# hmorimitsu/ptlflow

Measured on NVIDIA B200. Metric: frame-pairs/sec RAFT 1024x436 12-iter, higher is better.
Workload: dtype f16 storage, f32 accumulate/coordinates

## Files before the change

### include/ptlflow_b200.h

```cpp
#ifndef PTLFLOW_B200_H_
#define PTLFLOW_B200_H_

#include <stddef.h>
#include <stdint.h>

#ifdef __cplusplus
extern "C" {
#endif

#if defined(__GNUC__)
#define PFB_API __attribute__((visibility("default")))
#else
#define PFB_API
#endif

typedef void* pfb_stream;

typedef enum { PFB_F32 = 0, PFB_F16 = 1, PFB_BF16 = 2 } pfb_dtype;

typedef enum {
  PFB_OK = 0,
  PFB_ERR_ARG = -1,
  PFB_ERR_CUDA = -2,
  PFB_ERR_UNSUPPORTED = -3
// ... 156 lines not shown
} pfb_raft_weights;

typedef struct {
  void* const* pyramid;
  const void* fmap1;
  void* net;
  const void* inp;
  float* coords;
  float* flow_up;
  float* flow_small;
  void* workspace;
  size_t workspace_bytes;
  const void* attention;
  float agg_gamma;
} pfb_raft_buffers;

PFB_API size_t pfb_raft_workspace_bytes(const pfb_raft_cfg* cfg);
PFB_API int pfb_raft_refine(const pfb_raft_cfg* cfg, const pfb_raft_weights* w, const pfb_raft_buffers* buf,
                    pfb_stream stream);
PFB_API int pfb_raft_update_iter(const pfb_raft_cfg* cfg, const pfb_raft_weights* w, const pfb_raft_buffers* buf,
                         const void* corr, void* mask_out, pfb_stream stream);

PFB_API int pfb_preprocess_frames(const void* images, void* out, int B, int H, int W, int Hp, int Wp, int pad_top,
                                  int pad_left, int out_channels, pfb_dtype dtype, pfb_stream stream);
PFB_API size_t pfb_instance_norm_workspace_bytes(int B, int C);
PFB_API int pfb_instance_norm_act(const void* x, void* y, const void* residual, void* workspace, int B, int H, int W, int C,
                                  float eps, int relu, pfb_dtype dtype, pfb_stream stream);
PFB_API int pfb_instance_norm_apply(const void* x, void* y, const void* residual, void* workspace, int B, int H, int W, int C,
                                    float eps, int relu, pfb_dtype dtype, pfb_stream stream);
PFB_API int pfb_flow_conv7x7(const float* flow, const void* wpack, const float* bias, void* out, int out_stride, int out_offset,
                             int B, int H, int W, pfb_dtype dtype, pfb_stream stream);
PFB_API int pfb_first_conv7x7s2(const void* x, const void* wpack, const float* bias, void* out, double* stats, int N, int H, int W,
                                int relu, pfb_dtype dtype, pfb_stream stream);
PFB_API int pfb_bias_act(const void* x, const float* bias, const void* residual, void* y, void* workspace, int B, int H, int W,
                         int C, int relu, pfb_dtype dtype, pfb_stream stream);

#define PFB_KERNEL_CLASSES 12
PFB_API unsigned long long pfb_launch_count(int kernel_class);
PFB_API int pfb_profile_enable(int on);
PFB_API int pfb_profile_collect(double* ms, unsigned long long* n, int len);

#ifdef __cplusplus
}
#endif
#endif
```

### ptlflow_b200/_lib.py

```python
from __future__ import annotations

import ctypes as C
import threading
import os
from typing import Optional

import torch

_PKG = os.path.dirname(os.path.abspath(__file__))
LIB_PATH = os.path.join(_PKG, "lib", "libptlflow_b200.so")

PFB_MAX_LEVELS = 8
PFB_MAX_SRC = 4

F32, F16, BF16 = 0, 1, 2
_DTYPES = {torch.float32: F32, torch.float16: F16, torch.bfloat16: BF16}

EPI_LINEAR, EPI_RELU, EPI_GRU_ZR, EPI_GRU_Q, EPI_FLOW, EPI_RELU_APPEND_FLOW, EPI_AXPY, EPI_LINEAR_F32 = range(8)

(L_CONVC1, L_CONVC2, L_CONVF1, L_CONVF2, L_CONV, L_GRU_ZR1, L_GRU_Q1, L_GRU_ZR2, L_GRU_Q2,
 L_FLOW1, L_FLOW2, L_MASK1, L_MASK2, L_AGG_V, L_FLOW2T,
 L_CTX_ZR1, L_CTX_Q1, L_CTX_ZR2, L_CTX_Q2, L_GRUX_ZR1, L_GRUX_Q1, L_GRUX_ZR2, L_GRUX_Q2, L_CONVC2F2, L_COUNT) = range(25)


# ... 59 lines not shown
    "pfb_corr_volume_build": (_I, [_P, _P, _PP, _I, _I, _I, _I, _I, _I, _I, _S]),
    "pfb_corr_volume_build_ex": (_I, [_P, _P, _PP, _I, _I, _I, _I, _I, _I, _I, C.c_float, _I, _I, _S]),
    "pfb_corr_level_bytes": (C.c_size_t, [_I, _I, _I, _I, _I]),
    "pfb_corr_lookup": (_I, [_PP, _P, _P, _I, _I, _I, _I, _I, _I, _I, _I, _I, _S]),
    "pfb_corr_lookup_ex": (_I, [_PP, C.POINTER(C.c_int), C.POINTER(C.c_int), _P, _P, _I, _I, _I, _I, _I, _I, _I, _I, _I, _S]),
    "pfb_corr_level_bytes_tiled": (C.c_size_t, [_I, _I, _I, _I, _I, _I]),
    "pfb_corr_volume_build_tiled": (_I, [_P, _P, _PP, _I, _I, _I, _I, _I, _I, _I, C.c_float, _I, _S]),
    "pfb_corr_lookup_tiled": (_I, [_PP, _P, _P, _I, _I, _I, _I, _I, _I, _I, _I, _I, _S]),
    "pfb_corr_lookup_onthefly": (_I, [_P, _PP, _P, _P, _I, _I, _I, _I, _I, _I, _I, _I, _I, _I, _S]),
    "pfb_corr_lookup_onthefly_tc_workspace_bytes": (C.c_size_t, [_I, _I, _I]),
    "pfb_corr_lookup_onthefly_tc": (_I, [_P, _PP, _P, _P, _P, _I, _I, _I, _I, _I, _I, _I, _I, _S]),
    "pfb_alt_corr_forward": (_I, [_P, _P, _P, _P, _I, _I, _I, _I, _I, _I, _I, _I, _I, _S]),
    "pfb_avg_pool2x2_nhwc": (_I, [_P, _P, _I, _I, _I, _I, _I, _S]),
    "pfb_conv2d": (_I, [C.POINTER(ConvParams), _S]),
    "pfb_pack_conv_weight": (_I, [_P, _P, _I, _I, _I, _I, _I, _I, _I, _I, _S]),
    "pfb_pack_bias": (_I, [_P, _P, _I, _I, _I, _S]),
    "pfb_pack_conv_weight_kmajor": (_I, [_P, _P, _I, _I, _I, _I, _I, _I, C.POINTER(C.c_int), _I, _I, _I, _I, _S]),
    "pfb_convex_upsample": (_I, [_P, _P, _P, _P, _I, _I, _I, _I, _I, _I, _I, _I, _S]),
    "pfb_upflow8": (_I, [_P, _P, _P, _I, _I, _I, _I, _I, _I, _I, _S]),
    "pfb_softmax_rows": (_I, [_P, C.c_size_t, _I, _I, _S]),
    "pfb_transpose_pm": (_I, [_P, _P, _I, _I, _I, _I, _I, _S]),
    "pfb_flow_tap_gather": (_I, [_P, _I, _P, _P, _P, _I, _I, _I, _S]),
    "pfb_context_split": (_I, [_P, _P, _P, _I, _I, _I, _I, _I, _I, _S]),
    "pfb_init_coords": (_I, [_P, _P, _I, _I, _I, _S]),
    "pfb_forward_interpolate": (_I, [_P, _P, _I, _I, _I, _S]),
    "pfb_raft_workspace_bytes": (C.c_size_t, [C.POINTER(RaftCfg)]),
    "pfb_raft_refine": (_I, [C.POINTER(RaftCfg), C.POINTER(RaftWeights), C.POINTER(RaftBuffers), _S]),
    "pfb_preprocess_frames": (_I, [_P, _P, _I, _I, _I, _I, _I, _I, _I, _I, _I, _S]),
    "pfb_instance_norm_workspace_bytes": (C.c_size_t, [_I, _I]),
    "pfb_instance_norm_act": (_I, [_P, _P, _P, _P, _I, _I, _I, _I, C.c_float, _I, _I, _S]),
    "pfb_instance_norm_apply": (_I, [_P, _P, _P, _P, _I, _I, _I, _I, C.c_float, _I, _I, _S]),
    "pfb_flow_conv7x7": (_I, [_P, _P, _P, _P, _I, _I, _I, _I, _I, _I, _S]),
    "pfb_first_conv7x7s2": (_I, [_P, _P, _P, _P, _P, _I, _I, _I, _I, _I, _S]),
    "pfb_bias_act": (_I, [_P, _P, _P, _P, _P, _I, _I, _I, _I, _I, _I, _S]),
    "pfb_launch_count": (C.c_ulonglong, [_I]),
    "pfb_profile_enable": (_I, [_I]),
    "pfb_profile_collect": (_I, [C.POINTER(C.c_double), C.POINTER(C.c_ulonglong), _I]),
    "pfb_raft_update_iter": (_I, [C.POINTER(RaftCfg), C.POINTER(RaftWeights), C.POINTER(RaftBuffers), _P, _P, _S]),
}


class LibraryMissing(RuntimeError):
    pass


def load() -> C.CDLL:
    global _lib
    if _lib is not None:
        return _lib
    if not os.path.exists(LIB_PATH):
        raise LibraryMissing(
            f"{LIB_PATH} not found: the ptlflow_b200 hot path is hand-written CUDA and has no fallback. "
            "Build it with `python -m ptlflow_b200.csrc.build` (needs nvcc, no GPU required to compile)."
        )
    lib = C.CDLL(LIB_PATH)
    for name, (res, args) in SIGNATURES.items():
        fn = getattr(lib, name)
        fn.restype = res
        fn.argtypes = args
    _lib = lib
    return lib


def check(rc: int, what: str = "") -> None:
    if rc != 0:
        msg = load().pfb_last_error().decode(errors="replace")
# ... 64 lines not shown
```

### ptlflow_b200/csrc/build.py

```python
from __future__ import annotations

import hashlib
import os
import subprocess
import sys
from concurrent.futures import ThreadPoolExecutor

HERE = os.path.dirname(os.path.abspath(__file__))
PKG = os.path.dirname(HERE)
ROOT = os.path.dirname(PKG)
LIB_DIR = os.path.join(PKG, "lib")
OBJ_DIR = os.path.join(HERE, "build")
LIB_PATH = os.path.join(LIB_DIR, "libptlflow_b200.so")

SOURCES = ["misc.cu", "prof.cu", "corr.cu", "conv_simt.cu", "refine.cu", "conv_umma.cu", "corr_umma.cu", "corr_tiled.cu", "corr_onthefly_umma.cu", "conv_special.cu", "tmap.cu", "encoder.cu", "first_conv.cu"]
NVCC_FLAGS = [
    "-gencode", "arch=compute_100a,code=sm_100a",
    "-O3", "-lineinfo", "-std=c++17",
    "-Xcompiler", "-fPIC", "-Xcompiler", "-fvisibility=hidden",
    "--expt-relaxed-constexpr",
]


def _nvcc() -> str:
    for cand in (os.environ.get("NVCC"), "/usr/local/cuda/bin/nvcc", "nvcc"):
        if cand and (os.path.isabs(cand) and os.path.exists(cand) or not os.path.isabs(cand)):
            return cand
    return "nvcc"


def _digest() -> str:
    h = hashlib.sha256()
    for name in sorted(os.listdir(HERE)) + [os.path.join(ROOT, "include", "ptlflow_b200.h")]:
        path = name if os.path.isabs(name) else os.path.join(HERE, name)
        if path.endswith((".cu", ".cuh", ".h", "build.py")):
            with open(path, "rb") as f:
                h.update(name.encode() + b"\0" + f.read())
    return h.hexdigest()


def build(force: bool = False, verbose: bool = False) -> str:
    os.makedirs(LIB_DIR, exist_ok=True)
    os.makedirs(OBJ_DIR, exist_ok=True)
    stamp = os.path.join(LIB_DIR, "build.stamp")
    digest = _digest()
    if not force and os.path.exists(LIB_PATH) and os.path.exists(stamp) and open(stamp).read().strip() == digest:
        return LIB_PATH
    nvcc = _nvcc()
# ... 28 lines not shown
```

### ptlflow_b200/csrc/encoder.cu

```cuda
#include <algorithm>

#include <stdlib.h>

#include "common.cuh"

namespace pfb {

template <typename T>
__global__ void preprocess_frames_kernel(const T* __restrict__ img, T* __restrict__ out, int B, int H, int W, int Hp,
                                         int Wp, int pad_top, int pad_left, int OC) {
  const size_t total = (size_t)2 * B * Hp * Wp;
  for (size_t idx = blockIdx.x * (size_t)blockDim.x + threadIdx.x; idx < total; idx += (size_t)gridDim.x * blockDim.x) {
    int x = (int)(idx % Wp);
    size_t t = idx / Wp;
    int y = (int)(t % Hp);
    int n = (int)(t / Hp);
    const int f = n / B, b = n - f * B;
    int sy = y - pad_top, sx = x - pad_left;
    sy = sy < 0 ? 0 : (sy >= H ? H - 1 : sy);
    sx = sx < 0 ? 0 : (sx >= W ? W - 1 : sx);
    const T* src = img + (((size_t)b * 2 + f) * 3) * H * W + (size_t)sy * W + sx;
    T* o = out + idx * OC;
#pragma unroll
    for (int c = 0; c < 3; ++c) {
// ... 91 lines not shown
    }
  }
  if (pl < lanes && (!pow2 || (threadIdx.x & 31) < c8n)) {
#pragma unroll
    for (int k = 0; k < 8; ++k) {
      atomicAdd(&acc[8 * co + k], s[k]);
      atomicAdd(&acc[C + 8 * co + k], q[k]);
    }
  }
  __syncthreads();
  for (int i = threadIdx.x; i < 2 * C; i += blockDim.x) {
    const int c = i % C, which = i / C;
    atomicAdd(stats + ((size_t)b * C + c) * 2 + which, (double)acc[i]);
  }
}

template <typename T>
__device__ __forceinline__ void store8(T* p, const float (&f)[8]) {
  uint4 u;
  T* h = reinterpret_cast<T*>(&u);
#pragma unroll
  for (int i = 0; i < 8; ++i) h[i] = from_f32<T>(f[i]);
  *reinterpret_cast<uint4*>(p) = u;
}
template <>
__device__ __forceinline__ void store8<float>(float* p, const float (&f)[8]) {
  reinterpret_cast<float4*>(p)[0] = make_float4(f[0], f[1], f[2], f[3]);
  reinterpret_cast<float4*>(p)[1] = make_float4(f[4], f[5], f[6], f[7]);
}

template <typename T>
__global__ void __launch_bounds__(256) affine_act_kernel(const T* __restrict__ x, const double* __restrict__ stats,
                                                         const float* __restrict__ bias, const T* __restrict__ residual,
                                                         T* __restrict__ y, int HW, int C, float eps, int relu, int pix_per_block) {
  const int b = blockIdx.y;
  const int c8n = C / 8;
  const int lanes = blockDim.x / c8n;
  const int co = threadIdx.x % c8n, pl = threadIdx.x / c8n;
  __shared__ float2 ss_sm[512];
  for (int c = threadIdx.x; c < C; c += blockDim.x) {
    float2 v = make_float2(1.f, bias ? __ldg(bias + c) : 0.f);
    if (stats) {
      const double2 sq = *reinterpret_cast<const double2*>(stats + ((size_t)b * C + c) * 2);
      const double mean = sq.x / HW;
      double var = sq.y / HW - mean * mean;
      var = var < 0 ? 0 : var;
      const float rstd = rsqrtf((float)var + eps);
      v = make_float2(rstd, (float)(-mean) * rstd);
    }
    ss_sm[c] = v;
  }
  __syncthreads();
  if (pl >= lanes) return;
  float sc[8], sh[8];
#pragma unroll
  for (int k = 0; k < 8; ++k) {
    sc[k] = ss_sm[8 * co + k].x;
    sh[k] = ss_sm[8 * co + k].y;
  }
  const int p0 = blockIdx.x * pix_per_block;
  const int p1 = min(p0 + pix_per_block, HW);
  const size_t base = (size_t)b * HW * C + 8 * co;
#pragma unroll 4
  for (int p = p0 + pl; p < p1; p += lanes) {
    const size_t off = base + (size_t)p * C;
    float v[8], r[8];
    load8<T>(x + off, v);
    if (residual) load8<T>(residual + off, r);
#pragma unroll
    for (int k = 0; k < 8; ++k) {
      float o = fmaf(v[k], sc[k], sh[k]);
      if (relu) o = fmaxf(o, 0.f);
      if (residual) o = fmaxf(r[k] + o, 0.f);
      v[k] = o;
    }
    store8<T>(y + off, v);
  }
}

template <typename T>
__global__ void __launch_bounds__(256) inorm_fused_kernel(const T* __restrict__ x, const T* __restrict__ residual, T* __restrict__ y,
                                                          double* __restrict__ stats, unsigned* __restrict__ counters, int B, int HW, int C,
                                                          float eps, int relu, int G, int ipw) {
  extern __shared__ float acc[];
  const int iw = blockIdx.x / G, g = blockIdx.x - iw * G;
  const int c8n = C / 8;
  const int lanes = blockDim.x / c8n;
  const int co = threadIdx.x % c8n, pl = threadIdx.x / c8n;
  const int slice = (HW + G - 1) / G;
  const int p0 = g * slice, p1 = min(p0 + slice, HW);
  const bool pow2 = (c8n & (c8n - 1)) == 0 && c8n <= 32 && (blockDim.x % c8n) == 0;
  for (int b = iw; b < B; b += ipw) {
    for (int i = threadIdx.x; i < 2 * C; i += blockDim.x) acc[i] = 0.f;
    __syncthreads();
    const size_t base = (size_t)b * HW * C + 8 * co;
    float s[8], q[8];
#pragma unroll
    for (int k = 0; k < 8; ++k) s[k] = q[k] = 0.f;
    if (pl < lanes) {
#pragma unroll 4
      for (int p = p0 + pl; p < p1; p += lanes) {
        float v[8];
        load8<T>(x + base + (size_t)p * C, v);
#pragma unroll
        for (int k = 0; k < 8; ++k) {
          s[k] += v[k];
// ... 77 lines not shown

extern "C" PFB_API int pfb_preprocess_frames(const void* images, void* out, int B, int H, int W, int Hp, int Wp, int pad_top,
                                             int pad_left, int out_channels, pfb_dtype dtype, pfb_stream stream) {
  PFB_CHECK_ARG(images && out, "preprocess_frames: null pointer");
  PFB_CHECK_ARG(out_channels >= 3 && out_channels <= 16, "preprocess_frames: out_channels=%d (3..16)", out_channels);
  PFB_CHECK_ARG(dtype_ok(dtype) && B > 0 && H > 0 && W > 0 && Hp >= H && Wp >= W && pad_top >= 0 && pad_left >= 0 &&
                    pad_top + H <= Hp && pad_left + W <= Wp,
                "preprocess_frames: bad geometry %dx%d -> %dx%d (+%d,+%d)", H, W, Hp, Wp, pad_top, pad_left);
  cudaStream_t s = as_stream(stream);
  size_t total = (size_t)2 * B * Hp * Wp;
  unsigned blocks = (unsigned)std::min<size_t>(ceil_div_sz(total, 256), (size_t)sm_count() * 16);
  ProfScope prof(KC_MISC, s);
  if (dtype != PFB_F32 && out_channels == 4 && pad_left == 0 && Wp == W && W % 8 == 0 &&
      ((reinterpret_cast<uintptr_t>(images) | reinterpret_cast<uintptr_t>(out)) & 15) == 0 && ((size_t)H * W) % 8 == 0) {
    blocks = (unsigned)std::min<size_t>(ceil_div_sz(total / 8, 256), (size_t)sm_count() * 16);
    if (dtype == PFB_F16) preprocess_frames_vec8_kernel<__half><<<blocks, 256, 0, s>>>((const __half*)images, (__half*)out, B, H, W, Hp, pad_top);
    else preprocess_frames_vec8_kernel<__nv_bfloat16><<<blocks, 256, 0, s>>>((const __nv_bfloat16*)images, (__nv_bfloat16*)out, B, H, W, Hp, pad_top);
    PFB_LAUNCH_CHECK();
    return PFB_OK;
  }
  PFB_DISPATCH_DTYPE(dtype, T, {
    preprocess_frames_kernel<T><<<blocks, 256, 0, s>>>((const T*)images, (T*)out, B, H, W, Hp, Wp, pad_top, pad_left, out_channels);
  });
  PFB_LAUNCH_CHECK();
  return PFB_OK;
}

extern "C" PFB_API size_t pfb_instance_norm_workspace_bytes(int B, int C) {
  return (size_t)B * C * (2 * sizeof(double) + sizeof(float2));
}

template <typename T>
static int launch_affine(const void* x, const double* stats, const float* bias, const void* residual, void* y, int B, int HW, int C,
                         float eps, int relu, cudaStream_t s) {
  const int ppb = HW >= 8192 ? 512 : (HW >= 1024 ? 128 : 32);
  dim3 grid(ceil_div(HW, ppb), B);
  affine_act_kernel<T><<<grid, 256, 0, s>>>((const T*)x, stats, bias, (const T*)residual, (T*)y, HW, C, eps, relu, ppb);
  PFB_LAUNCH_CHECK();
  return PFB_OK;
}

extern "C" PFB_API int pfb_instance_norm_act(const void* x, void* y, const void* residual, void* workspace, int B, int H, int W,
                                             int C, float eps, int relu, pfb_dtype dtype, pfb_stream stream) {
  PFB_CHECK_ARG(x && y && workspace, "instance_norm_act: null pointer");
  PFB_CHECK_ARG(dtype_ok(dtype) && B > 0 && H > 0 && W > 0 && C > 0 && C % 8 == 0 && C <= 512,
                "instance_norm_act: bad shape (C=%d must be a multiple of 8, <= 512)", C);
  cudaStream_t s = as_stream(stream);
  const int HW = H * W;
  double* stats = reinterpret_cast<double*>(workspace);
  PFB_CUDA(cudaMemsetAsync(stats, 0, (size_t)B * C * 2 * sizeof(double) + (size_t)B * sizeof(unsigned), s));
  PFB_CHECK_ARG(B <= 65535, "instance_norm_act: batch too large");
  {
    static const int env_fused = getenv("PFB_INORM_FUSED") ? atoi(getenv("PFB_INORM_FUSED")) : 0;
    const size_t image_bytes = (size_t)HW * C * dtype_size(dtype);
    if (env_fused && dtype != PFB_F32 && C <= 256 && (256 % (C / 8) == 0 || C / 8 <= 32) && HW >= 1024) {
      const size_t per_image = image_bytes * (residual ? 3 : 2);
      int ipw = (int)std::max<size_t>(1, std::min<size_t>((size_t)B, (size_t)(60u << 20) / std::max<size_t>(per_image, 1)));
      const int sms = sm_count();
      if (ipw > sms / 2) ipw = sms / 2;
      const int G = std::max(1, sms / ipw);
      unsigned* counters = reinterpret_cast<unsigned*>(stats + (size_t)B * C * 2);
      ProfScope prof(KC_ENC_AFFINE, s);
      PFB_DISPATCH_DTYPE(dtype, T, {
        inorm_fused_kernel<T><<<ipw * G, 256, 2 * C * sizeof(float), s>>>((const T*)x, (const T*)residual, (T*)y, stats, counters, B, HW, C, eps,
                                                                        relu, G, ipw);
      });
      PFB_LAUNCH_CHECK();
      return PFB_OK;
    }
  }
  const int threads = 256;
  static const int env_ppb = getenv("PFB_STATS_PPB") ? atoi(getenv("PFB_STATS_PPB")) : 0;
  const int ppb = env_ppb > 0 && HW >= 8192 ? env_ppb : (HW >= 65536 ? 1536 : (HW >= 8192 ? 768 : (HW >= 1024 ? 256 : 64)));
  dim3 grid(ceil_div(HW, ppb), B);
  {
    ProfScope prof(KC_ENC_STATS, s);
    PFB_DISPATCH_DTYPE(dtype, T, { inorm_stats_kernel<T><<<grid, threads, 2 * C * sizeof(float), s>>>((const T*)x, stats, HW, C, ppb); });
  }
  PFB_LAUNCH_CHECK();
  ProfScope prof(KC_ENC_AFFINE, s);
  PFB_DISPATCH_DTYPE(dtype, T, { return launch_affine<T>(x, stats, nullptr, residual, y, B, HW, C, eps, relu, s); });
  return PFB_OK;
}

extern "C" PFB_API int pfb_instance_norm_apply(const void* x, void* y, const void* residual, void* workspace, int B, int H, int W,
                                               int C, float eps, int relu, pfb_dtype dtype, pfb_stream stream) {
  PFB_CHECK_ARG(x && y && workspace, "instance_norm_apply: null pointer");
  PFB_CHECK_ARG(dtype_ok(dtype) && B > 0 && H > 0 && W > 0 && C > 0 && C % 8 == 0 && C <= 512 && B <= 65535,
                "instance_norm_apply: bad shape (C=%d must be a multiple of 8, <= 512)", C);
  cudaStream_t s = as_stream(stream);
  const int HW = H * W;
  double* stats = reinterpret_cast<double*>(workspace);
  ProfScope prof(KC_ENC_AFFINE, s);
  PFB_DISPATCH_DTYPE(dtype, T, { return launch_affine<T>(x, stats, nullptr, residual, y, B, HW, C, eps, relu, s); });
  return PFB_OK;
}

extern "C" PFB_API int pfb_bias_act(const void* x, const float* bias, const void* residual, void* y, void* workspace, int B, int H,
                                    int W, int C, int relu, pfb_dtype dtype, pfb_stream stream) {
  PFB_CHECK_ARG(x && y && workspace, "bias_act: null pointer");
  PFB_CHECK_ARG(dtype_ok(dtype) && B > 0 && H > 0 && W > 0 && C > 0 && C % 8 == 0 && C <= 512, "bias_act: bad shape (C=%d must be a multiple of 8, <= 512)", C);
  PFB_CHECK_ARG(B <= 65535, "bias_act: batch too large");
  cudaStream_t s = as_stream(stream);
  (void)workspace;
  ProfScope prof(KC_ENC_AFFINE, s);
  PFB_DISPATCH_DTYPE(dtype, T, { return launch_affine<T>(x, nullptr, bias, residual, y, B, H * W, C, 0.f, relu, s); });
  return PFB_OK;
}
```

### ptlflow_b200/models/raft/extractor.py

```python
from __future__ import annotations

import os
import threading

import torch
import torch.nn as nn
import torch.nn.functional as F

from ... import _lib, ops


def _norm(kind: str, channels: int, groups: int = 8) -> nn.Module:
    if kind == "batch":
        return nn.BatchNorm2d(channels)
    if kind == "instance":
        return nn.InstanceNorm2d(channels)
    if kind == "group":
        return nn.GroupNorm(num_groups=groups, num_channels=channels)
    if kind == "none":
        return nn.Identity()
    raise ValueError(f"unknown norm_fn {kind!r}")


class ResidualBlock(nn.Module):
# ... 30 lines not shown
        g = planes // 8
        self.norm1, self.norm2, self.norm3 = _norm(norm_fn, q, g), _norm(norm_fn, q, g), _norm(norm_fn, planes, g)
        self.downsample = None
        if stride != 1:
            self.norm4 = _norm(norm_fn, planes, g)
            self.downsample = nn.Sequential(nn.Conv2d(in_planes, planes, 1, stride=stride), self.norm4)

    def forward(self, x):
        y = self.relu(self.norm1(self.conv1(x)))
        y = self.relu(self.norm2(self.conv2(y)))
        y = self.relu(self.norm3(self.conv3(y)))
        if self.downsample is not None:
            x = self.downsample(x)
        return self.relu(x + y)


def _fold(conv: nn.Conv2d, norm: nn.Module, dtype, device):
    w = conv.weight.detach().to(device=device, dtype=torch.float32)
    b = conv.bias.detach().to(device=device, dtype=torch.float32) if conv.bias is not None else torch.zeros(w.shape[0], device=device)
    if isinstance(norm, nn.BatchNorm2d):
        s = norm.weight.detach().float().to(device) / torch.sqrt(norm.running_var.detach().float().to(device) + norm.eps)
        t = norm.bias.detach().float().to(device) - norm.running_mean.detach().float().to(device) * s
        w = w * s.view(-1, 1, 1, 1)
        b = b * s + t
    w = w.to(dtype).contiguous(memory_format=torch.channels_last)
    b = b.contiguous()
    if dtype == torch.float32:
        return w, b
    return w, b, b.to(dtype)


_NATIVE_CONV1 = bool(int(os.environ.get("PFB_NATIVE_CONV1", "1")))
_NATIVE_CONV2 = bool(int(os.environ.get("PFB_NATIVE_CONV2", "1")))
_CUDNN_FUSED_RELU = bool(int(os.environ.get("PFB_CUDNN_FUSED_RELU", "1")))
_prep_lock = threading.Lock()


def _conv_pm(x: torch.Tensor, wb, stride: int, padding: int) -> torch.Tensor:
    y = F.conv2d(x.permute(0, 3, 1, 2), wb[0], None, stride=stride, padding=padding)
    y = y.permute(0, 2, 3, 1)
    return y if y.is_contiguous() else y.contiguous()


class _Encoder(nn.Module):
    block = ResidualBlock
    widths = (64, 64, 96, 128)

    def __init__(self, output_dim: int = 128, norm_fn: str = "batch", dropout: float = 0.0) -> None:
        super().__init__()
        self.norm_fn = norm_fn
        w0, w1, w2, w3 = self.widths
        self.norm1 = _norm(norm_fn, w0, 8)
        self.conv1 = nn.Conv2d(3, w0, 7, stride=2, padding=3)
        self.relu1 = nn.ReLU(inplace=True)
        self.layer1 = self._stage(w0, w1, 1)
        self.layer2 = self._stage(w1, w2, 2)
        self.layer3 = self._stage(w2, w3, 2)
        self.conv2 = nn.Conv2d(w3, output_dim, 1)
        self.dropout = nn.Dropout2d(p=dropout) if dropout > 0 else None
        for m in self.modules():
            if isinstance(m, nn.Conv2d):
                nn.init.kaiming_normal_(m.weight, mode="fan_out", nonlinearity="relu")
            elif isinstance(m, (nn.BatchNorm2d, nn.InstanceNorm2d, nn.GroupNorm)) and m.weight is not None:
                nn.init.ones_(m.weight)
                nn.init.zeros_(m.bias)

    def _stage(self, cin: int, cout: int, stride: int) -> nn.Sequential:
        return nn.Sequential(self.block(cin, cout, self.norm_fn, stride=stride), self.block(cout, cout, self.norm_fn, stride=1))

    def _signature(self, dtype, device):
        return (dtype, str(device)) + tuple((p.data_ptr(), p._version) for p in self.parameters()) + \
            tuple((b.data_ptr(), b._version) for b in self.buffers())

    def _prepared(self, dtype, device):
        sig = self._signature(dtype, device)
        cache = getattr(self, "_prep_cache", None)
        if cache is not None and cache[0] == sig:
            return cache[1]
        with _prep_lock:
            cache = getattr(self, "_prep_cache", None)
            if cache is not None and cache[0] == sig:
                return cache[1]
            return self._prepare_locked(sig, dtype, device)

    def _prepare_locked(self, sig, dtype, device):
        prep = {"conv1": _fold(self.conv1, self.norm1, dtype, device), "conv2": _fold(self.conv2, nn.Identity(), dtype, device), "blocks": []}
        for layer in (self.layer1, self.layer2, self.layer3):
            for blk in layer:
                e = {"stride": blk.conv2.stride[0] if isinstance(blk, BottleneckBlock) else blk.conv1.stride[0]}
                names = ("conv1", "conv2", "conv3") if isinstance(blk, BottleneckBlock) else ("conv1", "conv2")
                for i, nme in enumerate(names, start=1):
                    e[nme] = _fold(getattr(blk, nme), getattr(blk, f"norm{i}"), dtype, device)
                if blk.downsample is not None:
                    e["down"] = _fold(blk.downsample[0], blk.downsample[1], dtype, device)
                prep["blocks"].append(e)
        if (_NATIVE_CONV1 and tuple(self.conv1.weight.shape) == (64, 3, 7, 7) and dtype in (torch.float16, torch.bfloat16)
                and self.norm_fn in ("instance", "batch", "none")):
            folded = _fold(self.conv1, self.norm1, torch.float32, device)
            prep["conv1_native"] = (ops.pack_first_conv(folded[0], dtype), folded[1])
        c2 = self.conv2
        if (_NATIVE_CONV2 and dtype in (torch.float16, torch.bfloat16) and tuple(c2.kernel_size) == (1, 1) and c2.in_channels % 64 == 0
                and c2.out_channels % 32 == 0 and c2.out_channels <= 1024):
            prep["conv2_native"] = ops.PackedConv([c2], dtype, device, src_channels=[c2.in_channels])
        torch.cuda.current_stream(device).synchronize()
        self._prep_cache = (sig, prep)
        return prep

    def forward_pm(self, x: torch.Tensor) -> torch.Tensor:
        if self.norm_fn not in ("instance", "batch", "none"):
            return ops.to_pixel_major(self.forward(x.permute(0, 3, 1, 2)))
        inst = self.norm_fn == "instance"
        prep = self._prepared(x.dtype, x.device)

        def conv_act(x, wb, stride, padding, relu=True, residual=None):
            if _CUDNN_FUSED_RELU and not inst and relu and residual is None and x.dtype != torch.float32:
                bh = wb[2] if len(wb) > 2 else wb[1].to(x.dtype)
                y = torch.cudnn_convolution_relu(x.permute(0, 3, 1, 2), wb[0], bh, (stride, stride), (padding, padding), (1, 1), 1)
                y = y.permute(0, 2, 3, 1)
                return y if y.is_contiguous() else y.contiguous()
            y = _conv_pm(x, wb, stride, padding)
            if inst:
                return ops.instance_norm_act(y, relu=relu, residual=residual, out=y)
            return ops.bias_act(y, wb[1], relu=relu, residual=residual, out=y)

        c1 = prep["conv1"]
        native_c1 = ("conv1_native" in prep and x.shape[-1] == 4 and tuple(self.conv1.weight.shape) == (64, 3, 7, 7) and x.dtype in (torch.float16, torch.bfloat16)
                     and x.shape[1] % 2 == 0 and x.shape[2] % 2 == 0)
        if native_c1:
            wpack, bias = prep["conv1_native"]
            if inst:
                ws = ops.instance_norm_workspace((x.shape[0], 0, 0, 64), x.device)
                y = ops.first_conv7x7s2(x, wpack, None, relu=False, stats_ws=ws)
                x = ops.instance_norm_apply(y, ws, relu=True, out=y)
            else:
                x = ops.first_conv7x7s2(x, wpack, bias, relu=True)
        elif x.shape[-1] != c1[0].shape[1]:
            key = ("conv1_pad", x.shape[-1])
            if key not in prep:
                w = torch.zeros((c1[0].shape[0], x.shape[-1]) + tuple(c1[0].shape[2:]), dtype=c1[0].dtype, device=c1[0].device)
                w[:, : c1[0].shape[1]] = c1[0]
                prep[key] = (w.contiguous(memory_format=torch.channels_last), c1[1])
            c1 = prep[key]
        if not native_c1:
            x = conv_act(x, c1, 2, 3)
        for e in prep["blocks"]:
            s = e["stride"]
            xs = conv_act(x, e["down"], s, 0, relu=False) if "down" in e else x
            if "conv3" in e:
                y = conv_act(x, e["conv1"], 1, 0)
                y = conv_act(y, e["conv2"], s, 1)
                x = conv_act(y, e["conv3"], 1, 0, relu=True, residual=xs)
            else:
                y = conv_act(x, e["conv1"], s, 1)
                x = conv_act(y, e["conv2"], 1, 1, relu=True, residual=xs)
        if "conv2_native" in prep and x.is_contiguous():
            packed = prep["conv2_native"]
            out = torch.empty(x.shape[:3] + (packed.Cout,), dtype=x.dtype, device=x.device)
            return ops.conv2d([x], packed, out, epilogue=_lib.EPI_LINEAR)
        y = _conv_pm(x, prep["conv2"], 1, 0)
        return ops.bias_act(y, prep["conv2"][1], relu=False, out=y)

    def forward(self, x):
        pair = isinstance(x, (tuple, list))
        if pair:
            n = x[0].shape[0]
            x = torch.cat(list(x), dim=0)
        x = self.relu1(self.norm1(self.conv1(x)))
        x = self.layer3(self.layer2(self.layer1(x)))
        x = self.conv2(x)
        if self.training and self.dropout is not None:
            x = self.dropout(x)
        return (x[:n], x[n:]) if pair else x


class BasicEncoder(_Encoder):
    block = ResidualBlock
    widths = (64, 64, 96, 128)


class SmallEncoder(_Encoder):
    block = BottleneckBlock
    widths = (32, 32, 64, 96)
```

### ptlflow_b200/ops.py

```python
from __future__ import annotations

import contextlib
import ctypes as C
import threading
from typing import List, Optional, Sequence

import torch

from . import _lib
from ._lib import check, dtype_code, load, ptr_array, require_cuda, stream_ptr


def to_pixel_major(x: torch.Tensor) -> torch.Tensor:
    return x.permute(0, 2, 3, 1).contiguous()


def coords_to_pixel_major(coords: torch.Tensor) -> torch.Tensor:
    return coords.permute(0, 2, 3, 1).float().contiguous()


def alloc_pyramid(B: int, H: int, W: int, levels: int, dtype: torch.dtype, device) -> List[torch.Tensor]:
    return [torch.empty((B * H * W, H >> l, W >> l), dtype=dtype, device=device) for l in range(levels)]


# ... 362 lines not shown
    a = torch.zeros(7, 128, 8, 8, dtype=torch.float32, device=w.device)
    wk = w.permute(2, 0, 3, 1)
    a[:, :, 1:8, 0:2] = wk
    a[:, :, 1:8, 2:4] = wk
    a = a.reshape(7, 128, 64).to(dtype)
    return a.reshape(7, 16, 8, 8, 8).permute(0, 1, 3, 2, 4).contiguous()


def flow_conv7x7(flow: torch.Tensor, wpack: torch.Tensor, bias: torch.Tensor, out: torch.Tensor, out_offset: int = 0) -> torch.Tensor:
    require_cuda(flow, "flow")
    B, H, W, _ = flow.shape
    with torch.cuda.device(flow.device):
        check(load().pfb_flow_conv7x7(flow.data_ptr(), wpack.data_ptr(), bias.data_ptr(), out.data_ptr(), out.shape[-1], out_offset,
                                      B, H, W, dtype_code(out.dtype), stream_ptr(flow.device)), "flow_conv7x7")
    return out


def first_conv7x7s2(x: torch.Tensor, wpack: torch.Tensor, bias: Optional[torch.Tensor], relu: bool,
                    stats_ws: Optional[torch.Tensor] = None) -> torch.Tensor:
    require_cuda(x, "x")
    N, H, W, C4 = x.shape
    if C4 != 4 or not x.is_contiguous():
        raise RuntimeError("first_conv7x7s2: expected contiguous [N,H,W,4] frames")
    out = torch.empty((N, H // 2, W // 2, 64), dtype=x.dtype, device=x.device)
    if stats_ws is not None:
        stats_ws[: N * 64 * 2].zero_()
    with torch.cuda.device(x.device):
        check(load().pfb_first_conv7x7s2(x.data_ptr(), wpack.data_ptr(), bias.data_ptr() if bias is not None else None, out.data_ptr(),
                                         stats_ws.data_ptr() if stats_ws is not None else None, N, H, W, int(relu), dtype_code(x.dtype),
                                         stream_ptr(x.device)), "first_conv7x7s2")
    return out


def instance_norm_workspace(x_shape, device) -> torch.Tensor:
    B, _, _, Cc = x_shape
    return _scratch(("inorm", str(device), B * Cc), B * Cc * 3, device)


def instance_norm_apply(x: torch.Tensor, ws: torch.Tensor, relu: bool = True, residual: Optional[torch.Tensor] = None, eps: float = 1e-5,
                        out: Optional[torch.Tensor] = None) -> torch.Tensor:
    require_cuda(x, "x")
    B, H, W, Cc = x.shape
    y = out if out is not None else torch.empty_like(x)
    with torch.cuda.device(x.device):
        check(load().pfb_instance_norm_apply(x.data_ptr(), y.data_ptr(), residual.data_ptr() if residual is not None else None,
                                             ws.data_ptr(), B, H, W, Cc, eps, int(relu), dtype_code(x.dtype), stream_ptr(x.device)),
              "instance_norm_apply")
    return y


def bias_act(x: torch.Tensor, bias: Optional[torch.Tensor], relu: bool = True, residual: Optional[torch.Tensor] = None,
             out: Optional[torch.Tensor] = None) -> torch.Tensor:
    require_cuda(x, "x")
    B, H, W, Cc = x.shape
    y = out if out is not None else torch.empty_like(x)
    ws = _scratch(("bias", str(x.device), Cc), Cc, x.device)
    if bias is not None:
        assert bias.dtype == torch.float32 and bias.numel() == Cc and bias.is_cuda
    with torch.cuda.device(x.device):
        check(load().pfb_bias_act(x.data_ptr(), bias.data_ptr() if bias is not None else None,
                                  residual.data_ptr() if residual is not None else None, y.data_ptr(), ws.data_ptr(), B, H, W, Cc,
                                  int(relu), dtype_code(x.dtype), stream_ptr(x.device)), "bias_act")
    return y
```

Before: 944.4.

## Add fused tcgen05 encoder 3x3 conv with deferred instance-norm application

Adds a persistent UMMA/TMA 3x3 conv kernel for the 64-channel encoder residual blocks (layer1). Where the input is still un-normalized, it applies the previous instance norm and ReLU in shared memory, and it accumulates output statistics in the epilogue. A join kernel then normalizes the block output and its residual in one pass. The goal is to remove the separate normalize passes and the generic conv launches for the encoder's full-resolution stage. In exchange it adds a large specialized kernel, fp32-to-double atomic statistics, and a more involved pipeline with more room for bugs.

```diff
diff --git a/include/ptlflow_b200.h b/include/ptlflow_b200.h
--- a/include/ptlflow_b200.h
+++ b/include/ptlflow_b200.h
@@ -212,6 +212,10 @@
                              int B, int H, int W, pfb_dtype dtype, pfb_stream stream);
 PFB_API int pfb_first_conv7x7s2(const void* x, const void* wpack, const float* bias, void* out, double* stats, int N, int H, int W,
                                 int relu, pfb_dtype dtype, pfb_stream stream);
+PFB_API int pfb_encoder_conv3x3(const void* x, const void* wpack, void* out, const double* in_stats, double* out_stats, int N, int H, int W,
+                                int C, float eps, pfb_dtype dtype, pfb_stream stream);
+PFB_API int pfb_instance_norm_join(const void* x, void* y, const void* residual, const void* workspace, const void* res_workspace,
+                                   int res_relu, int B, int H, int W, int C, float eps, int relu, pfb_dtype dtype, pfb_stream stream);
 PFB_API int pfb_bias_act(const void* x, const float* bias, const void* residual, void* y, void* workspace, int B, int H, int W,
                          int C, int relu, pfb_dtype dtype, pfb_stream stream);
 
diff --git a/ptlflow_b200/_lib.py b/ptlflow_b200/_lib.py
--- a/ptlflow_b200/_lib.py
+++ b/ptlflow_b200/_lib.py
@@ -115,6 +115,8 @@
     "pfb_instance_norm_apply": (_I, [_P, _P, _P, _P, _I, _I, _I, _I, C.c_float, _I, _I, _S]),
     "pfb_flow_conv7x7": (_I, [_P, _P, _P, _P, _I, _I, _I, _I, _I, _I, _S]),
     "pfb_first_conv7x7s2": (_I, [_P, _P, _P, _P, _P, _I, _I, _I, _I, _I, _S]),
+    "pfb_encoder_conv3x3": (_I, [_P, _P, _P, _P, _P, _I, _I, _I, _I, C.c_float, _I, _S]),
+    "pfb_instance_norm_join": (_I, [_P, _P, _P, _P, _P, _I, _I, _I, _I, _I, C.c_float, _I, _I, _S]),
     "pfb_bias_act": (_I, [_P, _P, _P, _P, _P, _I, _I, _I, _I, _I, _I, _S]),
     "pfb_launch_count": (C.c_ulonglong, [_I]),
     "pfb_profile_enable": (_I, [_I]),
diff --git a/ptlflow_b200/csrc/build.py b/ptlflow_b200/csrc/build.py
--- a/ptlflow_b200/csrc/build.py
+++ b/ptlflow_b200/csrc/build.py
@@ -13,7 +13,7 @@
 OBJ_DIR = os.path.join(HERE, "build")
 LIB_PATH = os.path.join(LIB_DIR, "libptlflow_b200.so")
 
-SOURCES = ["misc.cu", "prof.cu", "corr.cu", "conv_simt.cu", "refine.cu", "conv_umma.cu", "corr_umma.cu", "corr_tiled.cu", "corr_onthefly_umma.cu", "conv_special.cu", "tmap.cu", "encoder.cu", "first_conv.cu"]
+SOURCES = ["misc.cu", "prof.cu", "corr.cu", "conv_simt.cu", "refine.cu", "conv_umma.cu", "corr_umma.cu", "corr_tiled.cu", "corr_onthefly_umma.cu", "conv_special.cu", "tmap.cu", "encoder.cu", "first_conv.cu", "encoder_conv.cu"]
 NVCC_FLAGS = [
     "-gencode", "arch=compute_100a,code=sm_100a",
     "-O3", "-lineinfo", "-std=c++17",
diff --git a/ptlflow_b200/csrc/encoder.cu b/ptlflow_b200/csrc/encoder.cu
--- a/ptlflow_b200/csrc/encoder.cu
+++ b/ptlflow_b200/csrc/encoder.cu
@@ -147,31 +147,35 @@
 template <typename T>
 __global__ void __launch_bounds__(256) affine_act_kernel(const T* __restrict__ x, const double* __restrict__ stats,
                                                          const float* __restrict__ bias, const T* __restrict__ residual,
-                                                         T* __restrict__ y, int HW, int C, float eps, int relu, int pix_per_block) {
+                                                         const double* __restrict__ rstats, int rrelu, T* __restrict__ y, int HW, int C,
+                                                         float eps, int relu, int pix_per_block) {
   const int b = blockIdx.y;
   const int c8n = C / 8;
   const int lanes = blockDim.x / c8n;
   const int co = threadIdx.x % c8n, pl = threadIdx.x / c8n;
   __shared__ float2 ss_sm[512];
+  __shared__ float2 rss_sm[512];
+  auto inorm_ss = [&](const double* st, int c) {
+    const double2 sq = *reinterpret_cast<const double2*>(st + ((size_t)b * C + c) * 2);
+    const double mean = sq.x / HW;
+    double var = sq.y / HW - mean * mean;
+    var = var < 0 ? 0 : var;
+    const float rstd = rsqrtf((float)var + eps);
+    return make_float2(rstd, (float)(-mean) * rstd);
+  };
   for (int c = threadIdx.x; c < C; c += blockDim.x) {
-    float2 v = make_float2(1.f, bias ? __ldg(bias + c) : 0.f);
-    if (stats) {
-      const double2 sq = *reinterpret_cast<const double2*>(stats + ((size_t)b * C + c) * 2);
-      const double mean = sq.x / HW;
-      double var = sq.y / HW - mean * mean;
-      var = var < 0 ? 0 : var;
-      const float rstd = rsqrtf((float)var + eps);
-      v = make_float2(rstd, (float)(-mean) * rstd);
-    }
-    ss_sm[c] = v;
+    ss_sm[c] = stats ? inorm_ss(stats, c) : make_float2(1.f, bias ? __ldg(bias + c) : 0.f);
+    if (rstats) rss_sm[c] = inorm_ss(rstats, c);
   }
   __syncthreads();
   if (pl >= lanes) return;
-  float sc[8], sh[8];
+  float sc[8], sh[8], rsc[8], rsh[8];
 #pragma unroll
   for (int k = 0; k < 8; ++k) {
     sc[k] = ss_sm[8 * co + k].x;
     sh[k] = ss_sm[8 * co + k].y;
+    rsc[k] = rstats ? rss_sm[8 * co + k].x : 1.f;
+    rsh[k] = rstats ? rss_sm[8 * co + k].y : 0.f;
   }
   const int p0 = blockIdx.x * pix_per_block;
   const int p1 = min(p0 + pix_per_block, HW);
@@ -186,7 +190,11 @@
     for (int k = 0; k < 8; ++k) {
       float o = fmaf(v[k], sc[k], sh[k]);
       if (relu) o = fmaxf(o, 0.f);
-      if (residual) o = fmaxf(r[k] + o, 0.f);
+      if (residual) {
+        float rv = rstats ? fmaf(r[k], rsc[k], rsh[k]) : r[k];
+        if (rrelu) rv = fmaxf(rv, 0.f);
+        o = fmaxf(rv + o, 0.f);
+      }
       v[k] = o;
     }
     store8<T>(y + off, v);
@@ -330,10 +338,10 @@
 
 template <typename T>
 static int launch_affine(const void* x, const double* stats, const float* bias, const void* residual, void* y, int B, int HW, int C,
-                         float eps, int relu, cudaStream_t s) {
+                         float eps, int relu, cudaStream_t s, const double* rstats = nullptr, int rrelu = 0) {
   const int ppb = HW >= 8192 ? 512 : (HW >= 1024 ? 128 : 32);
   dim3 grid(ceil_div(HW, ppb), B);
-  affine_act_kernel<T><<<grid, 256, 0, s>>>((const T*)x, stats, bias, (const T*)residual, (T*)y, HW, C, eps, relu, ppb);
+  affine_act_kernel<T><<<grid, 256, 0, s>>>((const T*)x, stats, bias, (const T*)residual, rstats, rrelu, (T*)y, HW, C, eps, relu, ppb);
   PFB_LAUNCH_CHECK();
   return PFB_OK;
 }
@@ -394,6 +402,21 @@
   return PFB_OK;
 }
 
+extern "C" PFB_API int pfb_instance_norm_join(const void* x, void* y, const void* residual, const void* workspace, const void* res_workspace,
+                                              int res_relu, int B, int H, int W, int C, float eps, int relu, pfb_dtype dtype,
+                                              pfb_stream stream) {
+  PFB_CHECK_ARG(x && y && residual && workspace, "instance_norm_join: null pointer");
+  PFB_CHECK_ARG(dtype_ok(dtype) && B > 0 && H > 0 && W > 0 && C > 0 && C % 8 == 0 && C <= 512 && B <= 65535,
+                "instance_norm_join: bad shape (C=%d must be a multiple of 8, <= 512)", C);
+  cudaStream_t s = as_stream(stream);
+  ProfScope prof(KC_ENC_AFFINE, s);
+  PFB_DISPATCH_DTYPE(dtype, T, {
+    return launch_affine<T>(x, (const double*)workspace, nullptr, residual, y, B, H * W, C, eps, relu, s, (const double*)res_workspace,
+                            res_relu);
+  });
+  return PFB_OK;
+}
+
 extern "C" PFB_API int pfb_bias_act(const void* x, const float* bias, const void* residual, void* y, void* workspace, int B, int H,
                                     int W, int C, int relu, pfb_dtype dtype, pfb_stream stream) {
   PFB_CHECK_ARG(x && y && workspace, "bias_act: null pointer");
diff --git a/ptlflow_b200/csrc/encoder_conv.cu b/ptlflow_b200/csrc/encoder_conv.cu
--- /dev/null
+++ b/ptlflow_b200/csrc/encoder_conv.cu
@@ -0,0 +1,315 @@
+#include <stdlib.h>
+
+#include "umma.cuh"
+
+namespace pfb {
+using namespace sm100;
+
+constexpr int kEcC = 64;
+constexpr int kEcTapBytes = kEcC * 128;
+constexpr int kEcWBytes = 9 * kEcTapBytes;
+constexpr int kEcRowPx = 264;
+constexpr int kEcRowBytes = kEcRowPx * 128;
+constexpr int kEcSlots = 4;
+constexpr int kEcEpiWarps = 8;
+constexpr int kEcXfWarps = 4;
+constexpr int kEcThreads = (6 + kEcEpiWarps - 4 + kEcXfWarps) * 32;
+
+struct __align__(8) EcBars {
+  uint64_t full[kEcSlots];
+  uint64_t ready[kEcSlots];
+  uint64_t empty[kEcSlots];
+  uint64_t acc_full[2];
+  uint64_t acc_empty[2];
+  uint64_t w_full;
+  uint32_t tmem_base;
+  float2 ss[kEcC];
+};
+
+struct EcArgs {
+  const void* wpack;
+  void* out;
+  const double* in_stats;
+  double* out_stats;
+  int N, H, W;
+  int pairs, nseg, n_items, per_cta;
+  float eps;
+  int ab_fmt;
+};
+
+template <typename T>
+__global__ void __launch_bounds__(kEcThreads, 1) encoder_conv3x3_kernel(const __grid_constant__ CUtensorMap tmX,
+                                                                       const __grid_constant__ CUtensorMap tmXt, const EcArgs a) {
+  extern __shared__ __align__(1024) uint8_t smem_raw[];
+  uint8_t* smem = reinterpret_cast<uint8_t*>((reinterpret_cast<uintptr_t>(smem_raw) + 1023) & ~uintptr_t(1023));
+  uint8_t* smemW = smem;
+  uint8_t* smemX = smemW + kEcWBytes;
+  uint8_t* smemStage = smemX + kEcSlots * kEcRowBytes;
+  EcBars* bars = reinterpret_cast<EcBars*>(smemStage + kEcEpiWarps * 2048);
+  const int warp = threadIdx.x >> 5, lane = threadIdx.x & 31;
+  const bool xform = a.in_stats != nullptr;
+
+  if (threadIdx.x == 0) {
+    for (int s = 0; s < kEcSlots; ++s) {
+      mbar_init(&bars->full[s], 1);
+      mbar_init(&bars->ready[s], kEcXfWarps);
+      mbar_init(&bars->empty[s], 1);
+    }
+    for (int s = 0; s < 2; ++s) {
+      mbar_init(&bars->acc_full[s], 1);
+      mbar_init(&bars->acc_empty[s], kEcEpiWarps);
+    }
+    mbar_init(&bars->w_full, 1);
+    fence_barrier_init();
+  }
+  if (warp == 5) tmem_alloc<512>(&bars->tmem_base);
+  tc_fence_before();
+  __syncthreads();
+  tc_fence_after();
+  const uint32_t tmem_base = bars->tmem_base;
+  if (warp == 4 && lane == 0) {
+    prefetch_tmap(&tmX);
+    prefetch_tmap(&tmXt);
+    mbar_arrive_expect_tx(&bars->w_full, kEcWBytes);
+    asm volatile("cp.async.bulk.shared::cluster.global.mbarrier::complete_tx::bytes [%0], [%1], %2, [%3];" ::"r"(smem_u32(smemW)),
+                 "l"(a.wpack), "r"((uint32_t)kEcWBytes), "r"(smem_u32(&bars->w_full))
+                 : "memory");
+  }
+  pdl_wait();
+  pdl_trigger();
+
+  const int w0 = blockIdx.x * a.per_cta;
+  const int w1 = min(a.n_items, w0 + a.per_cta);
+  auto decode = [&](int w, int& n, int& y, int& x0) {
+    const int per_img = a.pairs * a.nseg;
+    n = w / per_img;
+    const int r = w - n * per_img;
+    const int q = r / a.nseg;
+    y = 2 * q;
+    x0 = (r - q * a.nseg) * 256;
+  };
+
+  if (warp == 4) {
+    int s = 0;
+    uint32_t ph = 0;
+    for (int w = w0; w < w1; ++w) {
+      int n, y, x0;
+      decode(w, n, y, x0);
+      for (int j = 0; j < 4; ++j) {
+        mbar_wait(&bars->empty[s], ph ^ 1);
+        if (elect_one()) {
+          uint8_t* dst = smemX + s * kEcRowBytes;
+          mbar_arrive_expect_tx(&bars->full[s], kEcRowBytes);
+          tma_load_4d(dst, &tmX, &bars->full[s], 0, x0 - 1, y - 1 + j, n);
+          tma_load_4d(dst + 256 * 128, &tmXt, &bars->full[s], 0, x0 + 255, y - 1 + j, n);
+        }
+        __syncwarp();
+        if (++s == kEcSlots) { s = 0; ph ^= 1; }
+      }
+    }
+  } else if (warp == 5) {
+    const uint32_t idesc = make_idesc_f16(64, 256, a.ab_fmt);
+    const uint32_t desc_hi = (1024u >> 4) | (1u << 14) | (2u << 29);
+    const uint32_t w_lo0 = ((smem_u32(smemW) & 0x3FFFF) >> 4) | (1u << 16);
+    mbar_wait(&bars->w_full, 0);
+    int s = 0, i = 0;
+    uint32_t ph = 0;
+    for (int w = w0; w < w1; ++w, ++i) {
+      const int acc_slot = i & 1;
+      mbar_wait(&bars->acc_empty[acc_slot], ((i >> 1) & 1) ^ 1);
+      tc_fence_after();
+      const uint32_t d0 = tmem_base + acc_slot * 256;
+      for (int j = 0; j < 4; ++j) {
+        mbar_wait(xform ? &bars->ready[s] : &bars->full[s], ph);
+        tc_fence_after();
+        if (elect_one()) {
+          const uint32_t x_lo = ((smem_u32(smemX + s * kEcRowBytes) & 0x3FFFF) >> 4) | (1u << 16);
+#pragma unroll
+          for (int r = 0; r < 2; ++r) {
+            const int ky = j - r;
+            if (ky < 0 || ky > 2) continue;
+            const uint32_t d = d0 + ((uint32_t)(16 * r) << 16);
+#pragma unroll
+            for (int kx = 0; kx < 3; ++kx) {
+#pragma unroll
+              for (int kk = 0; kk < 4; ++kk) {
+                const uint32_t al = w_lo0 + (uint32_t)(((ky * 3 + kx) * kEcTapBytes + kk * 32) >> 4);
+                const uint32_t bl = x_lo + (uint32_t)((kx * 128 + kk * 32) >> 4);
+                umma_f16_lohi(d, al, bl, desc_hi, idesc, (ky == 0 && kx == 0 && kk == 0) ? 0u : 1u);
+              }
+            }
+          }
+          umma_commit(&bars->empty[s]);
+        }
+        __syncwarp();
+        if (++s == kEcSlots) { s = 0; ph ^= 1; }
+      }
+      if (elect_one()) umma_commit(&bars->acc_full[acc_slot]);
+      __syncwarp();
+    }
+  } else if (warp >= 10) {
+    if (xform) {
+      const int t = threadIdx.x - 320;
+      int s = 0, n_cur = -1;
+      uint32_t ph = 0;
+      for (int w = w0; w < w1; ++w) {
+        int n, y, x0;
+        decode(w, n, y, x0);
+        if (n != n_cur) {
+          named_barrier_sync(2, 128);
+          if (t < kEcC) {
+            const double sum = a.in_stats[((size_t)n * kEcC + t) * 2], sq = a.in_stats[((size_t)n * kEcC + t) * 2 + 1];
+            const double hw = (double)a.H * a.W;
+            const double mean = sum / hw;
+            double var = sq / hw - mean * mean;
+            var = var < 0 ? 0 : var;
+            const float rstd = rsqrtf((float)var + a.eps);
+            bars->ss[t] = make_float2(rstd, (float)(-mean) * rstd);
+          }
+          named_barrier_sync(2, 128);
+          n_cur = n;
+        }
+        const int i_lo = x0 - 1 < 0 ? 1 - x0 : 0;
+        const int i_hi = min(258, a.W - (x0 - 1));
+        for (int j = 0; j < 4; ++j) {
+          mbar_wait(&bars->full[s], ph);
+          const int r = y - 1 + j;
+          if (r >= 0 && r < a.H) {
+            uint8_t* row = smemX + s * kEcRowBytes;
+            for (int e = i_lo * 8 + t; e < i_hi * 8; e += 128) {
+              const int px = e >> 3, k = e & 7;
+              const int c0 = 8 * (k ^ (px & 7));
+              uint4* p = reinterpret_cast<uint4*>(row + px * 128 + k * 16);
+              uint4 u = *p;
+              T* h = reinterpret_cast<T*>(&u);
+#pragma unroll
+              for (int q = 0; q < 8; ++q) {
+                const float2 ss = bars->ss[c0 + q];
+                h[q] = from_f32<T>(fmaxf(fmaf(to_f32(h[q]), ss.x, ss.y), 0.f));
+              }
+              *p = u;
+            }
+          }
+          fence_proxy_async();
+          __syncwarp();
+          if (lane == 0) mbar_arrive(&bars->ready[s]);
+          if (++s == kEcSlots) { s = 0; ph ^= 1; }
+        }
+      }
+    }
+  } else {
+    const int quarter = warp & 3, group = warp < 4 ? 0 : 1;
+    const int rsel = lane >> 4, co = 16 * quarter + (lane & 15);
+    uint8_t* stage = smemStage + (group * 4 + quarter) * 2048;
+    float ssum = 0.f, ssq = 0.f;
+    int n_cur = -1;
+    auto flush = [&]() {
+      if (a.out_stats && n_cur >= 0) {
+        atomicAdd(&a.out_stats[((size_t)n_cur * kEcC + co) * 2 + 0], (double)ssum);
+        atomicAdd(&a.out_stats[((size_t)n_cur * kEcC + co) * 2 + 1], (double)ssq);
+      }
+      ssum = 0.f;
+      ssq = 0.f;
+    };
+    int i = 0;
+    for (int w = w0; w < w1; ++w, ++i) {
+      int n, y, x0;
+      decode(w, n, y, x0);
+      if (n != n_cur) {
+        flush();
+        n_cur = n;
+      }
+      const int acc_slot = i & 1;
+      const bool row_ok = y + rsel < a.H;
+      const bool row1_ok = y + 1 < a.H;
+      mbar_wait(&bars->acc_full[acc_slot], (i >> 1) & 1);
+      tc_fence_after();
+      const uint32_t taddr = tmem_base + acc_slot * 256 + ((uint32_t)(quarter * 32) << 16);
+      T* obase = reinterpret_cast<T*>(a.out) + (((size_t)n * a.H + y) * a.W) * kEcC + 16 * quarter;
+#pragma unroll 1
+      for (int c = group; c < 8; c += 2) {
+        const int xb = x0 + 32 * c;
+        if (xb >= a.W) break;
+        uint32_t r[32];
+        tmem_ld_32x32(taddr + 32 * c, r);
+        tmem_ld_wait();
+        const int nv = a.W - xb;
+        T* st = reinterpret_cast<T*>(stage);
+#pragma unroll
+        for (int e = 0; e < 32; ++e) {
+          const float v = __uint_as_float(r[e]);
+          if (row_ok && e < nv) {
+            ssum += v;
+            ssq = fmaf(v, v, ssq);
+          }
+          st[e * 32 + lane] = from_f32<T>(v);
+        }
+        __syncwarp();
+#pragma unroll
+        for (int k = 0; k < 4; ++k) {
+          const int id = k * 32 + lane;
+          const int half = id & 1, px = (id >> 1) & 31, rr = id >> 6;
+          if (px < nv && (rr == 0 || row1_ok))
+            *reinterpret_cast<uint4*>(obase + ((size_t)rr * a.W + xb + px) * kEcC + half * 8) =
+                *reinterpret_cast<const uint4*>(stage + px * 64 + rr * 32 + half * 16);
+        }
+        __syncwarp();
+      }
+      tc_fence_before();
+      __syncwarp();
+      if (lane == 0) mbar_arrive(&bars->acc_empty[acc_slot]);
+    }
+    flush();
+  }
+  tc_fence_before();
+  __syncthreads();
+  if (warp == 5) tmem_dealloc<512>(tmem_base);
+}
+
+}
+
+using namespace pfb;
+
+extern "C" PFB_API int pfb_encoder_conv3x3(const void* x, const void* wpack, void* out, const double* in_stats, double* out_stats, int N,
+                                           int H, int W, int C, float eps, pfb_dtype dtype, pfb_stream stream) {
+  PFB_CHECK_ARG(x && wpack && out, "encoder_conv3x3: null pointer");
+  PFB_CHECK_ARG(dtype == PFB_F16 || dtype == PFB_BF16, "encoder_conv3x3: f16 / bf16 storage only (fp32 runs in cuDNN)");
+  PFB_CHECK_ARG(C == kEcC, "encoder_conv3x3: C=%d (only 64 -> 64 channels)", C);
+  PFB_CHECK_ARG(N > 0 && H > 0 && W > 0 && H <= 65535 && W <= 65535, "encoder_conv3x3: bad shape %dx%dx%d", N, H, W);
+  PFB_CHECK_ARG(((reinterpret_cast<uintptr_t>(x) | reinterpret_cast<uintptr_t>(out) | reinterpret_cast<uintptr_t>(wpack)) & 15) == 0,
+                "encoder_conv3x3: 16-byte alignment");
+  cudaStream_t s = as_stream(stream);
+  CUtensorMap tmX, tmXt;
+  {
+    const uint64_t dims[4] = {(uint64_t)kEcC, (uint64_t)W, (uint64_t)H, (uint64_t)N};
+    const uint64_t str[3] = {(uint64_t)kEcC * 2, (uint64_t)W * kEcC * 2, (uint64_t)H * W * kEcC * 2};
+    const uint32_t box[4] = {(uint32_t)kEcC, 256, 1, 1};
+    int rc = make_tensor_map(&tmX, x, dtype, 4, dims, str, box);
+    if (rc) return rc;
+    const uint32_t tail[4] = {(uint32_t)kEcC, (uint32_t)(kEcRowPx - 256), 1, 1};
+    rc = make_tensor_map(&tmXt, x, dtype, 4, dims, str, tail);
+    if (rc) return rc;
+  }
+  EcArgs a{};
+  a.wpack = wpack; a.out = out; a.in_stats = in_stats; a.out_stats = out_stats;
+  a.N = N; a.H = H; a.W = W;
+  a.pairs = ceil_div(H, 2);
+  a.nseg = ceil_div(W, 256);
+  a.n_items = N * a.pairs * a.nseg;
+  a.eps = eps;
+  a.ab_fmt = dtype == PFB_F16 ? 0 : 1;
+  int grid = sm_count();
+  if (grid > a.n_items) grid = a.n_items;
+  a.per_cta = ceil_div(a.n_items, grid);
+  grid = ceil_div(a.n_items, a.per_cta);
+  const size_t smem = kEcWBytes + (size_t)kEcSlots * kEcRowBytes + kEcEpiWarps * 2048 + sizeof(EcBars) + 1024;
+  ProfScope prof(KC_ENC_CONV1, s);
+  if (dtype == PFB_F16) {
+    PFB_CUDA(cudaFuncSetAttribute(encoder_conv3x3_kernel<__half>, cudaFuncAttributeMaxDynamicSharedMemorySize, (int)smem));
+    PFB_CUDA(launch_pdl(encoder_conv3x3_kernel<__half>, dim3(grid), dim3(kEcThreads), smem, s, tmX, tmXt, a));
+  } else {
+    PFB_CUDA(cudaFuncSetAttribute(encoder_conv3x3_kernel<__nv_bfloat16>, cudaFuncAttributeMaxDynamicSharedMemorySize, (int)smem));
+    PFB_CUDA(launch_pdl(encoder_conv3x3_kernel<__nv_bfloat16>, dim3(grid), dim3(kEcThreads), smem, s, tmX, tmXt, a));
+  }
+  return PFB_OK;
+}
diff --git a/ptlflow_b200/models/raft/extractor.py b/ptlflow_b200/models/raft/extractor.py
--- a/ptlflow_b200/models/raft/extractor.py
+++ b/ptlflow_b200/models/raft/extractor.py
@@ -86,6 +86,7 @@
 
 _NATIVE_CONV1 = bool(int(os.environ.get("PFB_NATIVE_CONV1", "1")))
 _NATIVE_CONV2 = bool(int(os.environ.get("PFB_NATIVE_CONV2", "1")))
+_NATIVE_ENCODER = bool(int(os.environ.get("PFB_NATIVE_ENCODER", "1")))
 _CUDNN_FUSED_RELU = bool(int(os.environ.get("PFB_CUDNN_FUSED_RELU", "1")))
 _prep_lock = threading.Lock()
 
@@ -147,6 +148,9 @@
                     e[nme] = _fold(getattr(blk, nme), getattr(blk, f"norm{i}"), dtype, device)
                 if blk.downsample is not None:
                     e["down"] = _fold(blk.downsample[0], blk.downsample[1], dtype, device)
+                elif (_NATIVE_ENCODER and self.norm_fn == "instance" and dtype in (torch.float16, torch.bfloat16)
+                      and isinstance(blk, ResidualBlock) and all(tuple(c.weight.shape) == (64, 64, 3, 3) for c in (blk.conv1, blk.conv2))):
+                    e["native3x3"] = tuple(ops.pack_encoder_conv3x3(c.weight.to(device), dtype) for c in (blk.conv1, blk.conv2))
                 prep["blocks"].append(e)
         if (_NATIVE_CONV1 and tuple(self.conv1.weight.shape) == (64, 3, 7, 7) and dtype in (torch.float16, torch.bfloat16)
                 and self.norm_fn in ("instance", "batch", "none")):
@@ -178,14 +182,15 @@
             return ops.bias_act(y, wb[1], relu=relu, residual=residual, out=y)
 
         c1 = prep["conv1"]
+        raw_ws = None
         native_c1 = ("conv1_native" in prep and x.shape[-1] == 4 and tuple(self.conv1.weight.shape) == (64, 3, 7, 7) and x.dtype in (torch.float16, torch.bfloat16)
                      and x.shape[1] % 2 == 0 and x.shape[2] % 2 == 0)
         if native_c1:
             wpack, bias = prep["conv1_native"]
             if inst:
-                ws = ops.instance_norm_workspace((x.shape[0], 0, 0, 64), x.device)
-                y = ops.first_conv7x7s2(x, wpack, None, relu=False, stats_ws=ws)
-                x = ops.instance_norm_apply(y, ws, relu=True, out=y)
+                ws = ops.instance_norm_workspace((x.shape[0], 0, 0, 64), x.device, tag="c1")
+                x = ops.first_conv7x7s2(x, wpack, None, relu=False, stats_ws=ws)
+                raw_ws = ws
             else:
                 x = ops.first_conv7x7s2(x, wpack, bias, relu=True)
         elif x.shape[-1] != c1[0].shape[1]:
@@ -199,6 +204,18 @@
             x = conv_act(x, c1, 2, 3)
         for e in prep["blocks"]:
             s = e["stride"]
+            if "native3x3" in e and x.is_contiguous():
+                w1, w2 = e["native3x3"]
+                ws1 = ops.instance_norm_workspace(x.shape, x.device, tag="e1")
+                ws2 = ops.instance_norm_workspace(x.shape, x.device, tag="e2")
+                y = ops.encoder_conv3x3(x, w1, in_ws=raw_ws, out_ws=ws1)
+                y = ops.encoder_conv3x3(y, w2, in_ws=ws1, out_ws=ws2)
+                x = ops.instance_norm_join(y, ws2, x, res_ws=raw_ws, res_relu=raw_ws is not None, out=y)
+                raw_ws = None
+                continue
+            if raw_ws is not None:
+                x = ops.instance_norm_apply(x, raw_ws, relu=True, out=x)
+                raw_ws = None
             xs = conv_act(x, e["down"], s, 0, relu=False) if "down" in e else x
             if "conv3" in e:
                 y = conv_act(x, e["conv1"], 1, 0)
@@ -207,6 +224,8 @@
             else:
                 y = conv_act(x, e["conv1"], s, 1)
                 x = conv_act(y, e["conv2"], 1, 1, relu=True, residual=xs)
+        if raw_ws is not None:
+            x = ops.instance_norm_apply(x, raw_ws, relu=True, out=x)
         if "conv2_native" in prep and x.is_contiguous():
             packed = prep["conv2_native"]
             out = torch.empty(x.shape[:3] + (packed.Cout,), dtype=x.dtype, device=x.device)
diff --git a/ptlflow_b200/ops.py b/ptlflow_b200/ops.py
--- a/ptlflow_b200/ops.py
+++ b/ptlflow_b200/ops.py
@@ -418,9 +418,51 @@
     return out
 
 
-def instance_norm_workspace(x_shape, device) -> torch.Tensor:
+def instance_norm_workspace(x_shape, device, tag=None) -> torch.Tensor:
     B, _, _, Cc = x_shape
-    return _scratch(("inorm", str(device), B * Cc), B * Cc * 3, device)
+    key = ("inorm", str(device), B * Cc) + ((tag,) if tag is not None else ())
+    return _scratch(key, B * Cc * 3, device)
+
+
+def pack_encoder_conv3x3(weight: torch.Tensor, dtype: torch.dtype) -> torch.Tensor:
+    if tuple(weight.shape) != (64, 64, 3, 3):
+        raise RuntimeError("pack_encoder_conv3x3: expected a [64,64,3,3] filter")
+    w = weight.detach().float().permute(2, 3, 0, 1).reshape(9, 64, 8, 8)
+    rows = torch.arange(64, device=w.device).view(64, 1).expand(64, 8)
+    phys = torch.arange(8, device=w.device).view(1, 8) ^ (rows % 8)
+    out = torch.empty_like(w)
+    out[:, rows, phys] = w
+    return out.to(dtype).contiguous()
+
+
+def encoder_conv3x3(x: torch.Tensor, wpack: torch.Tensor, in_ws: Optional[torch.Tensor] = None, out_ws: Optional[torch.Tensor] = None,
+                    eps: float = 1e-5) -> torch.Tensor:
+    require_cuda(x, "x")
+    N, H, W, Cc = x.shape
+    if not x.is_contiguous():
+        raise RuntimeError("encoder_conv3x3: expected a contiguous [N,H,W,64] tensor")
+    out = torch.empty_like(x)
+    if out_ws is not None:
+        out_ws[: N * Cc * 2].zero_()
+    with torch.cuda.device(x.device):
+        check(load().pfb_encoder_conv3x3(x.data_ptr(), wpack.data_ptr(), out.data_ptr(), in_ws.data_ptr() if in_ws is not None else None,
+                                         out_ws.data_ptr() if out_ws is not None else None, N, H, W, Cc, eps, dtype_code(x.dtype),
+                                         stream_ptr(x.device)), "encoder_conv3x3")
+    return out
+
+
+def instance_norm_join(x: torch.Tensor, ws: torch.Tensor, residual: torch.Tensor, res_ws: Optional[torch.Tensor] = None,
+                       res_relu: bool = False, relu: bool = True, eps: float = 1e-5, out: Optional[torch.Tensor] = None) -> torch.Tensor:
+    require_cuda(x, "x")
+    require_cuda(residual, "residual")
+    assert residual.shape == x.shape
+    B, H, W, Cc = x.shape
+    y = out if out is not None else torch.empty_like(x)
+    with torch.cuda.device(x.device):
+        check(load().pfb_instance_norm_join(x.data_ptr(), y.data_ptr(), residual.data_ptr(), ws.data_ptr(),
+                                            res_ws.data_ptr() if res_ws is not None else None, int(res_relu), B, H, W, Cc, eps, int(relu),
+                                            dtype_code(x.dtype), stream_ptr(x.device)), "instance_norm_join")
+    return y
 
 
 def instance_norm_apply(x: torch.Tensor, ws: torch.Tensor, relu: bool = True, residual: Optional[torch.Tensor] = None, eps: float = 1e-5,
```

New measurement: 915.4, median of 6. 0.969x the previous value.
